# FauxFaux/quadrs

Hardware: AMD Instinct MI355X
Metric: Msamples/s through shift->FIR->FFT chain (higher is better)
Workload: dtype f32

## Files before the change

quadrs_amd/csrc/qd_chain.h:

```cpp
#pragma once

#include "qd_device.h"
#include "qd_geometry.h"

namespace qd {

#ifdef QD_STAMP
#define QD_STAMP_DECL unsigned long long st_prev = 0, st_acc[8] = {0, 0, 0, 0, 0, 0, 0, 0}, st_row[4] = {0, 0, 0, 0}; unsigned st_tiles = 0;
#define QD_STAMP_ROW(k) do { unsigned long long t_; asm volatile("s_memtime %0\n\ts_waitcnt lgkmcnt(0)" : "=s"(t_) :: "memory"); st_row[k] += t_ - st_prev; st_acc[0] += t_ - st_prev; st_prev = t_; } while (0)
#define QD_STAMP_START() do { asm volatile("s_memtime %0\n\ts_waitcnt lgkmcnt(0)" : "=s"(st_prev) :: "memory"); } while (0)
#define QD_STAMP_AT(k) do { unsigned long long t_; asm volatile("s_memtime %0\n\ts_waitcnt lgkmcnt(0)" : "=s"(t_) :: "memory"); st_acc[k] += t_ - st_prev; st_prev = t_; } while (0)
#define QD_STAMP_FLUSH() do { if (P.stamps && (threadIdx.x & 63) == 0 && threadIdx.x < 1024) { unsigned w_ = threadIdx.x >> 6; for (int k_ = 0; k_ < 8; ++k_) atomicAdd(&P.stamps[w_ * 8 + k_], st_acc[k_]); if (w_ == 1) for (int k_ = 0; k_ < 4; ++k_) atomicAdd(&P.stamps[129 + k_], st_row[k_]); if (w_ == 0) for (int k_ = 0; k_ < 4; ++k_) atomicAdd(&P.stamps[133 + k_], st_row[k_]); if (w_ == 0) atomicAdd(&P.stamps[128], (unsigned long long)st_tiles); } } while (0)
#define QD_STAMP_TILE() do { ++st_tiles; } while (0)
#else
#define QD_STAMP_DECL
#define QD_STAMP_START()
#define QD_STAMP_AT(k)
#define QD_STAMP_FLUSH()
#define QD_STAMP_TILE()
#define QD_STAMP_ROW(k)
#endif

#ifdef QD_BAKED_TAPS_LIST
constexpr float kBakedTapTable[] = {QD_BAKED_TAPS_LIST};
// ... 60 lines not shown
template <class GeoT>
__device__ __forceinline__ uint8_t glyph_of(const ChainParams &P, float nm) {
    if constexpr (GeoT::kFixed) return glyph_code(nm, P.rmin, P.rmax, P.gstep, P.rgstep);
    else return glyph_code_ieee(nm, P.rmin, P.rmax, P.gstep);
}

template <class GeoT>
__device__ __forceinline__ float2 win_mul(const ChainParams &P, uint32_t k, float2 v) {
    if constexpr (GeoT::kWindow) { const float wv = P.window[k]; v.x = v.x * wv; v.y = v.y * wv; }
    return v;
}
template <class GeoT>
__device__ __forceinline__ float win_mul(const ChainParams &P, uint32_t k, float v) {
    if constexpr (GeoT::kWindow) v = v * P.window[k];
    return v;
}


typedef float v2f __attribute__((ext_vector_type(2)));

template <uint32_t W_, uint32_t S_, uint32_t D_, uint32_t T_, uint32_t G_, uint32_t FIRB_ = 8, uint32_t FIRR_ = 1, uint32_t PAD_ = 1, uint32_t BATCH_ = 1,
          uint32_t FLAGS_ = 0>
struct FixedGeo {
    static constexpr bool kFixed = true;
    static constexpr bool kRows = false;
    static constexpr FixedRules R = fixed_rules(W_, S_, D_, T_, G_, FIRB_, FIRR_, PAD_, BATCH_, FLAGS_);
    static constexpr uint32_t kFlags = FLAGS_;
    static constexpr bool kWindow = (FLAGS_ & kGeoWindow) != 0;
    static constexpr uint32_t DpP = R.DpP;
    static constexpr uint32_t plane_floats = R.plane_floats;
    static constexpr bool planar_geometry = R.planar_geometry;
    static constexpr bool baked_request = R.baked_request;
    static constexpr uint32_t kBatch = R.kBatch;
    static constexpr uint32_t kFirBlock = R.kFirBlock;
    static constexpr bool kFirTile4 = R.kFirTile4;
    static constexpr uint32_t kFirTile = R.kFirTile;
    static constexpr uint32_t PD = R.PD;
    static constexpr uint32_t pshift = R.pshift;
    __device__ __forceinline__ explicit FixedGeo(const ChainParams &) {}
    static constexpr uint32_t W = W_, S = S_, D = D_, T = T_, G = G_;
    static constexpr uint32_t G_ct = G_, W_ct = W_;
    static constexpr uint32_t logW = R.logW;
    static constexpr uint32_t kPad = R.kPad;
    static constexpr uint32_t Dp = R.Dp;
    static constexpr uint32_t dshift = R.dshift;
    static constexpr uint32_t dmagic = R.dmagic;
    static constexpr uint32_t c = R.c;
    static constexpr uint32_t a0 = R.a0, b0 = R.b0;
    static constexpr uint32_t T_fast = R.T_fast;
    static constexpr uint32_t a1 = R.a1, b1 = R.b1;
    static constexpr uint32_t log_base = R.log_base;
    static constexpr uint32_t base_len = R.base_len;
    static constexpr uint32_t layers = R.layers;
    static constexpr bool kHalfTile = R.kHalfTile;
    static constexpr uint32_t kHalfOut = R.kHalfOut;
    static constexpr uint32_t kHalfRaw = R.kHalfRaw;
    static constexpr uint32_t lds_raw_elems_std = R.lds_raw_elems_std;
    static constexpr uint32_t kNtrunc = R.kNtrunc;
    static constexpr bool kShared = R.kShared;
    static constexpr bool split_ok(uint32_t nt) { return R.split_ok(nt); }
    static constexpr bool helper_ok(uint32_t nt) { return R.helper_ok(nt); }
    static constexpr bool split_ok_shared(uint32_t nt) { return R.split_ok_shared(nt); }
    static constexpr bool kPairFir = R.kPairFir;
    static constexpr bool kUnrolledShared = R.kUnrolledShared;
    static constexpr bool kPackedTile = R.kPackedTile;
    static constexpr bool kPlanar = R.kPlanar;
    static constexpr bool kBakedTaps = R.kBakedTaps;
    static constexpr uint32_t lds_raw_elems = R.lds_raw_elems;
};

struct DynGeo {
    static constexpr bool kFixed = false;
    static constexpr bool kRows = false;
    static constexpr bool kWindow = false;
    static constexpr uint32_t kBatch = 1;
    static constexpr uint32_t kFlags = 0, G_ct = 1, W_ct = 1;
    static constexpr bool kPlanar = false, kBakedTaps = false, kPairFir = false, kUnrolledShared = false, kPackedTile = false, kHalfTile = false;
    static constexpr uint32_t kHalfOut = 0, kHalfRaw = 0;
    static constexpr uint32_t DpP = 0, plane_floats = 0;
    static constexpr bool kShared = false;
    static constexpr uint32_t kFirTile = 1;
    static constexpr bool split_ok(uint32_t) { return false; }
    static constexpr bool helper_ok(uint32_t) { return false; }
    static constexpr bool split_ok_shared(uint32_t) { return false; }
    uint32_t W, S, D, T, G, logW, Dp, kPad, dshift, dmagic, PD, pshift, a0, b0, T_fast, a1, b1, log_base, base_len, layers, lds_raw_elems;
    __device__ __forceinline__ explicit DynGeo(const ChainParams &P)
        : W(P.W), S(P.S), D(P.D), T(P.T), G(P.G), logW(P.logW), Dp(P.Dp), kPad(P.Dp - P.D), dshift(P.dshift), dmagic(P.dmagic), PD(P.D), pshift(P.dshift),
          a0(P.a0), b0(P.b0), T_fast(P.T_fast), a1(P.a1), b1(P.b1), log_base(P.log_base), base_len(P.base_len),
          layers(P.layers), lds_raw_elems(P.lds_raw_elems) {}
};

struct WinGeo : DynGeo {
    static constexpr bool kWindow = true;
    __device__ __forceinline__ explicit WinGeo(const ChainParams &P) : DynGeo(P) {}
};

struct RowGeo : DynGeo {
    static constexpr bool kRows = true;
    __device__ __forceinline__ explicit RowGeo(const ChainParams &P) : DynGeo(P) {}
};


struct TileGeo {
    uint64_t w0, n_start;
    uint64_t r0;
    int64_t row0_off;
    int32_t slab_lo0, slab_hi0;
    uint32_t n_rows;
// ... 919 lines not shown
            float2 *d = fbp + (size_t)chunk * 4 * cols + i;
            float2 s0 = d[0];
            float2 s1 = cmul(d[cols], tw[3 * i]);
            float2 s2 = cmul(d[2 * cols], tw[3 * i + 1]);
            float2 s3 = cmul(d[3 * cols], tw[3 * i + 2]);
            bf4(s0, s1, s2, s3);
            d[0] = s0; d[cols] = s1; d[2 * cols] = s2; d[3 * cols] = s3;
        }
        tw += 3 * cols;
        cols *= 4;
        log_cols += 2;
    }
    wsync();
    if constexpr (PART == 3) return;
    const uint64_t wrel = pw0 - P.out_window0;
    const uint32_t n_out_s = pg << geo.logW;
    if (P.epi == 2) {
        constexpr uint32_t K = KB ? KB : (GeoT::kFixed ? (GeoT::G_ct * GeoT::W_ct + 63) / 64 : 1);
        wave_bucket_epilogue_fn<GeoT, K>(P, geo, fbp, pw0, pg, lane);
    } else if (P.epi == 4) {
        wave_mark_epilogue_fn<GeoT>(P, geo, [&](uint32_t o) { return fbp[o]; }, reinterpret_cast<uint8_t *>(P.out) + wrel, pg, lane);
    } else {
        float *outf = reinterpret_cast<float *>(P.out) + (wrel << geo.logW);
        uint8_t *outb = reinterpret_cast<uint8_t *>(P.out) + (wrel << geo.logW);
        for (uint32_t o = lane; o < n_out_s; o += 64) {
            const float2 xv = fbp[o ^ (geo.W >> 1)];
            const float nm = norm_ref(xv);
            if (P.epi == 0) outf[o] = nm;
            else outb[o] = glyph_of<GeoT>(P, nm);
        }
    }
}

template <class GeoT, bool HAS_FIR>
constexpr bool defer_fft_ok(uint32_t nt) {
    if constexpr (!GeoT::kFixed) return false;
    else return GeoT::R.defer_fft_ok(HAS_FIR, nt);
}

template <class GeoT, bool HAS_FIR>
constexpr bool quad_fft_ok(uint32_t nt) {
    if constexpr (!GeoT::kFixed) return false;
    else return GeoT::R.quad_fft_ok(HAS_FIR, nt);
}

template <int FMT, int NT, class GeoT>
constexpr bool fast_p1_ok(int rch, bool whole, bool aligned) {
    if constexpr (!GeoT::kFixed) return false;
    else return GeoT::R.fast_p1_ok(NT, FmtTraits<FMT>::SPL, (uint64_t)rch, whole, aligned);
}

template <int FMT, int NCO, class GeoT, bool HAS_FIR, int RCH, bool WHOLE, bool ALIGNED, int LB, int NT = kThreads>
__global__ __launch_bounds__(NT, LB) void k_chain(const ChainParams P) {
    using FT = FmtTraits<FMT>;
    using Vec = typename FT::Vec;
    constexpr int SPL = FT::SPL;
    constexpr bool HAS_SHIFT = NCO != 0;
    const GeoT geo(P);

    extern __shared__ __attribute__((aligned(16))) char smem[];
    float2 *raw = reinterpret_cast<float2 *>(smem);
    constexpr bool kDefer = defer_fft_ok<GeoT, HAS_FIR>((uint32_t)NT);
    constexpr bool kQuadFft = quad_fft_ok<GeoT, HAS_FIR>((uint32_t)NT);
    constexpr uint32_t kSlots = GeoT::kBatch;
    constexpr uint32_t kBatch = kDefer ? 1u : GeoT::kBatch;
    constexpr uint32_t kLutElems = (FMT == 1 || FMT == 2) ? 256u : 0u;
    float2 *fb0 = raw + geo.lds_raw_elems;
    float2 *twl = fb0 + (size_t)kSlots * geo.G * geo.W;
    float *tapl = reinterpret_cast<float *>(twl + geo.W);
    float *lut = tapl + ((GeoT::kBakedTaps && NT == 256) ? 0u : ((geo.T + 3) & ~3u));
    float2 *dec = reinterpret_cast<float2 *>(lut + kLutElems);
    float2 *trc = dec + ((geo.G - 1) * geo.S + geo.W);
    uint32_t *bmeta = reinterpret_cast<uint32_t *>(GeoT::kShared ? trc + ((geo.G - 1) * geo.S + geo.W) : dec);
    uint32_t *wq = bmeta + 4 * kSlots;

    const uint32_t tid = threadIdx.x;
    const uint32_t W = geo.W, logW = geo.logW, S = geo.S, D = geo.D, T = geo.T, Dp = geo.Dp;


    constexpr bool kReloadLane = HAS_SHIFT && ((GeoT::kFixed && GeoT::kFirTile > 1) || !GeoT::kFixed);
    constexpr bool kFastP1 = fast_p1_ok<FMT, NT, GeoT>(RCH, WHOLE, ALIGNED);
    constexpr bool kHalf = GeoT::kHalfTile;
    static_assert(!kHalf || (kFastP1 && defer_fft_ok<GeoT, HAS_FIR>((uint32_t)NT)), "half-window tiles: row-aligned phase 1 and the deferred FFT");
    static_assert((GeoT::kFlags & kGeoWindow) == 0 || (GeoT::kFixed && family_of(GeoT::kFlags) == kFamChain), "kGeoWindow: a plan-time build of k_chain");
    static_assert(!GeoT::kWindow || HAS_FIR || GeoT::kFixed, "WinGeo: behind a lowpass only (without one DynGeo tests the pointer)");
    uint32_t half = 0;
    LaneRot lr[SPL];
    auto load_lane_rot = [&](uint32_t first) {
#pragma unroll
        for (int u = 0; u < SPL; ++u) {
            uint32_t j = first + u;
            double2 cs = P.jtab[j];
            lr[u].jf = (double)j;
            lr[u].c = cs.x;
            lr[u].s = cs.y;
        }
    };
// ... 34 lines not shown
        asm volatile("" : "+s"(mx));
        const uint64_t dyn_base = 2 * walk_step;
        if (got + dyn_base < xcd_limit(mx)) return (uint64_t)mx * n8 + dyn_base + got;
#pragma unroll 1
        for (uint32_t k = 1; k < 8; ++k) {
            const uint32_t xx = (mx + k) & 7u;
            const uint64_t lim = xcd_limit(xx);
            if (lim <= dyn_base) continue;
            const unsigned long long i = atomicAdd(&P.work[16 * xx], 1ull);
            if (i + dyn_base < lim) return (uint64_t)xx * n8 + dyn_base + i;
        }
        return n_tiles;
    };
    uint64_t tile, tile_n;
    tile = walk_tile(walk_local);
    tile_n = walk_tile(walk_local + walk_step);
    TileGeo tg = tile_geo<FMT, NT>(P, geo, tile, n_tiles);
    Vec pf[RCH];
    if constexpr (!GeoT::kRows) {
    if (tg.valid) {
#pragma unroll
        for (int i = 0; i < RCH; ++i) pf[i] = fetch_row<FMT, NT, ALIGNED, (GeoT::kFlags & kGeoNtLoads) != 0>(P, tg, (uint32_t)i < tg.n_rows ? i : tg.n_rows - 1, tid);
    }
    }

#ifdef QD_WGTIME
    unsigned long long wg_t0 = __builtin_amdgcn_s_memrealtime();
#endif
    double rt_touch = 0.0;
    uint32_t dpar = 0, dprev_gcnt = 0;
    uint64_t dprev_w0 = 0;
    bool dprev_valid = false;
    auto wave_fft_epilogue = [&](float2 *fbp, uint64_t pw0, uint32_t pg) { wave_fft_epilogue_fn<GeoT>(P, geo, twl, fbp, pw0, pg, tid); };
    auto parks_norms = [](uint32_t epi) { return epi == 2 || (!GeoT::kFixed && epi == 4); };
    uint32_t quad_gen = 0;
    auto quad_fft_epilogue = [&](float2 *fbp, uint64_t pw0, uint32_t v) {
        uint32_t lane = tid & 63u;
        asm volatile("" : "+v"(lane));
        auto wsync = [] { __builtin_amdgcn_fence(__ATOMIC_ACQ_REL, "wavefront"); __builtin_amdgcn_wave_barrier(); };
        const uint32_t Wq = geo.W >> 2, base = geo.base_len;
        float2 *sub = fbp + (size_t)v * Wq;
        for (uint32_t t = lane; t < Wq / base; t += 64) {
            float2 *d = sub + (size_t)t * base;
            if (base == 16) {
                float2 x[16];
#pragma unroll
                for (int i = 0; i < 16; ++i) x[i] = d[i];
                bf16(x, P.tw16_1, P.tw16_2, P.tw16_3, P.root2);
#pragma unroll
                for (int i = 0; i < 16; ++i) d[i] = x[i];
            } else {
                float2 x[8];
#pragma unroll
                for (int i = 0; i < 8; ++i) x[i] = d[i];
                bf8(x, P.root2);
#pragma unroll
                for (int i = 0; i < 8; ++i) d[i] = x[i];
            }
        }
        uint32_t cols = base, log_cols = geo.log_base;
        const float2 *tw = twl;
        for (uint32_t layer = 0; layer + 1 < geo.layers; ++layer) {
            wsync();
            for (uint32_t t = lane; t < Wq / 4; t += 64) {
                const uint32_t chunk = t >> log_cols, i = t & (cols - 1);
                float2 *d = sub + (size_t)chunk * 4 * cols + i;
// ... 147 lines not shown
#pragma unroll
                for (int i = 0; i < RCH; ++i) cur[i] = pf[i];
                TileGeo ng = tg;
                uint32_t rbase = r + RCH;
                if (rbase >= tg.n_rows) {
                    const TileGeo t2 = tile_geo<FMT, NT>(P, geo, tile_n, n_tiles);
                    if (t2.valid) { ng = t2; rbase = 0; rt_pf = prefetch_rowtab<HAS_SHIFT>(P, t2, tid); } else { rbase = tg.n_rows - 1; }
                }
#pragma unroll
                for (int i = 0; i < RCH; ++i)
                    pf[i] = fetch_row<FMT, NT, ALIGNED, (GeoT::kFlags & kGeoNtLoads) != 0>(P, ng, rbase + i < ng.n_rows ? rbase + i : ng.n_rows - 1, tid);
                RowBase rb[RCH];
#pragma unroll
                for (int i = 0; i < RCH; ++i) {
                    rb[i] = RowBase{};
                    if constexpr (HAS_SHIFT) { if (r + i < tg.n_rows) rb[i] = load_rowbase(P, tg.r0 + r + i); }
                }
#pragma unroll
                for (int i = 0; i < RCH; ++i)
                    if (r + i < tg.n_rows) process_row_any<FMT, NT, NCO>(P, geo, tg, r + i, tid, cur[i], rb[i], lr, lane_pad, lut, raw);
            }
        }
        QD_STAMP_AT(0);
        __syncthreads();
        QD_STAMP_AT(1);

        __builtin_amdgcn_s_setprio(1);
        if constexpr (kDefer) {
            constexpr uint32_t GW = GeoT::G_ct * GeoT::W_ct, GWP = kHalf ? GeoT::kHalfOut : GW, FL = GeoT::kPackedTile ? GWP / 2 : GWP;
            float2 *fb_cur = fb0 + (size_t)dpar * GW, *fb_prev = fb0 + (size_t)(dpar ^ 1u) * GW;
            const uint32_t n_out_d = kHalf ? GWP : (g_cnt << logW);
            const uint32_t log_width_d = 2 * geo.layers;
            const uint32_t k_first = kHalf ? half * GWP : 0u;
            if (tid < FL) {
                if constexpr (GeoT::kPackedTile) {
                    const uint32_t o0 = tid * 2;
                    if (o0 < n_out_d) {
                        const uint32_t g = kHalf ? 0u : (o0 >> logW), k0 = kHalf ? k_first + o0 : (o0 & (W - 1));
                        uint32_t jm[2];
#pragma unroll
                        for (int r = 0; r < 2; ++r) { const uint32_t j2 = (W - (k0 + r)) * D + T / 2; jm[r] = j2 < T ? j2 : T; }
                        float2 full[2], snp[2];
                        const uint32_t q0 = kHalf ? o0 : g * S + k0;
                        if ((tid >> 8) & 1u) fir_tiled2_pk<GeoT, 1>(raw + (q0 * D + GeoT::kPad * (q0 / 2)), tapl, full, jm, snp); else fir_tiled2_pk<GeoT, 0>(raw + (q0 * D + GeoT::kPad * (q0 / 2)), tapl, full, jm, snp);
#pragma unroll
                        for (int r = 0; r < 2; ++r) {
                            const uint32_t k = k0 + r;
                            const uint32_t xx = k & ((1u << log_width_d) - 1), yy = k >> log_width_d;
                            fb_cur[(g << logW) + yy + (rev4(xx, geo.layers) << geo.log_base)] = win_mul<GeoT>(P, k, jm[r] < T ? snp[r] : full[r]);
                        }
                    }
                } else if (tid < n_out_d) {
                    const uint32_t g = kHalf ? 0u : (tid >> logW), k = kHalf ? k_first + tid : (tid & (W - 1));
                    uint32_t jmax = (W - k) * D + T / 2;
                    if (jmax > T) jmax = T;
                    const float2 *rp = raw + (size_t)((kHalf ? tid : g * S + k) + geo.a0) * Dp;
                    const float2 v = QD_DBG(P, 2) ? rp[0] : fir_pair<GeoT>(rp, jmax, tapl);
                    const uint32_t xx = k & ((1u << log_width_d) - 1), yy = k >> log_width_d;
                    fb_cur[(g << logW) + yy + (rev4(xx, geo.layers) << geo.log_base)] = win_pair(k, v);
                }
            } else if (kHalf && half != 0) {
            } else if (kQuadFft && !one_wave_sink(P.epi)) {
                if ((tid >> 6) < FL / 64 + 4 && dprev_valid) {
                    __builtin_amdgcn_s_setprio(3);
                    quad_fft_epilogue(fb_prev, dprev_w0, (tid >> 6) - FL / 64);
                }
            } else if ((tid >> 6) == FL / 64 && dprev_valid) {
                __builtin_amdgcn_s_setprio(3);
                wave_fft_epilogue(fb_prev, dprev_w0, dprev_gcnt);
            }
            QD_STAMP_AT(2);
            if constexpr (kHalf) {
                if (half == 0) {
                    __syncthreads();
                    QD_STAMP_AT(3);
                    half = 1;
                    rt_touch += rt_pf;
                    continue;
                }
                half = 0;
            }
            if (dyn && tid == 0) {
                const uint64_t t2 = claim_resolve(claim);
                wq[0] = (uint32_t)t2; wq[1] = (uint32_t)(t2 >> 32);
            }
            const TileGeo tg_nx = tile_geo<FMT, NT>(P, geo, tile_n, n_tiles);
            __syncthreads();
            QD_STAMP_AT(3);
            dprev_w0 = w0; dprev_gcnt = g_cnt; dprev_valid = true; dpar ^= 1u;
            tile = tile_n;
            if (dyn) tile_n = ((uint64_t)__builtin_amdgcn_readfirstlane(wq[1]) << 32) | __builtin_amdgcn_readfirstlane(wq[0]);
            else { walk_local += walk_step; tile_n = walk_tile(walk_local + walk_step); }
            rt_touch += rt_pf;
            tg = tg_nx;
            QD_STAMP_TILE();
            continue;
        }
        float2 *fb = fb0 + (size_t)bslot * geo.G * geo.W;
        const uint32_t n_out = g_cnt << logW;
        const uint32_t log_width = 2 * geo.layers;
        const bool cf32_out = !GeoT::kFixed && P.epi == 3;
        const uint32_t c_half = T - T / 2;
        const uint32_t ntrunc = c_half ? (c_half + D - 1) / D - 1 : 0;
        bool shared;
        if constexpr (GeoT::kFixed) shared = GeoT::kShared; else shared = HAS_FIR && S < W && ntrunc <= S && !QD_DBG(P, 2) && P.epi != 3;
        if constexpr (!GeoT::kFixed || GeoT::kShared) if (shared) {
            const uint32_t Q = (g_cnt - 1) * S + W;
            if constexpr (GeoT::kFixed && GeoT::kFirTile > 1) {
                constexpr int R = (int)GeoT::kFirTile;
                for (uint32_t q0 = tid * R; q0 < Q; q0 += NT * R) {
                    uint32_t jm[R];
#pragma unroll
                    for (int r = 0; r < R; ++r) {
                        const uint32_t qi = q0 + r;
                        jm[r] = T;
                        if (qi + ntrunc >= W) {
                            const uint32_t g = (qi - (W - ntrunc)) / S, k = qi - g * S;
                            if (k < W && g < g_cnt) { const uint32_t j2 = (W - k) * D + T / 2; if (j2 < T) jm[r] = j2; }
                        }
                    }
                    float2 full[R], snp[R];
                    fir_tiled<R, GeoT>(raw + (q0 * D + GeoT::kPad * (q0 / R)), jm, tapl, full, snp);
// ... 290 lines not shown
                asm volatile("" : "+v"(tt));
                reinterpret_cast<uint8_t *>(P.out)[wrel + tt] = (GeoT::kFixed || P.epi == 2) ? (first < second ? 0 : 1) : (mark ? 1 : 0);
            }
        } else if (GeoT::kFixed && P.epi == 4) {
            uint32_t ln = tid & 63u;
            asm volatile("" : "+v"(ln));
            wave_mark_epilogue_fn<GeoT>(P, geo, [&](uint32_t o) { return fbs[o]; }, reinterpret_cast<uint8_t *>(P.out) + wrel, n_out_s >> logW, ln,
                                        __builtin_amdgcn_readfirstlane(tid >> 6), NT / 64);
        } else {
            float *outf = reinterpret_cast<float *>(P.out) + (wrel << logW);
            uint8_t *outb = reinterpret_cast<uint8_t *>(P.out) + (wrel << logW);
            for (uint32_t o = tid; o < n_out_s; o += NT) {
                uint32_t oi = o;
                asm volatile("" : "+v"(oi));
                const float2 xv = fbs[oi ^ (W >> 1)];
                const float nm = QD_DBG(P, 8) ? xv.x : norm_ref(xv);
                uint32_t oo = o;
                asm volatile("" : "+v"(oo));
                if (QD_DBG(P, 16)) { asm volatile("" :: "v"(nm)); continue; }
                if (P.epi == 0) outf[oo] = nm;
                else outb[oo] = glyph_of<GeoT>(P, nm);
            }
        }
        }
        rt_touch += rt_pf;
        QD_STAMP_AT(6);
        if (parks_norms(P.epi)) __syncthreads();
        QD_STAMP_AT(7);
        QD_STAMP_TILE();
        tg = tg_next;
    }
    if constexpr (kDefer) {
        constexpr uint32_t GW = GeoT::G_ct * GeoT::W_ct, GWP = kHalf ? GeoT::kHalfOut : GW, FL = GeoT::kPackedTile ? GWP / 2 : GWP;
        if (kQuadFft && !one_wave_sink(P.epi)) {
            if (dprev_valid && (tid >> 6) >= FL / 64 && (tid >> 6) < FL / 64 + 4) quad_fft_epilogue(fb0 + (size_t)(dpar ^ 1u) * GW, dprev_w0, (tid >> 6) - FL / 64);
        } else
        if (dprev_valid && (tid >> 6) == FL / 64) wave_fft_epilogue(fb0 + (size_t)(dpar ^ 1u) * GW, dprev_w0, dprev_gcnt);
    }
    if (dyn && tid == 0) {
        if (atomicAdd(&P.work[16 * 8], 1ull) == (unsigned long long)gridDim.x - 1) {
#pragma unroll
            for (int x = 0; x <= 8; ++x) P.work[16 * x] = 0;
        }
    }
    QD_STAMP_FLUSH();
#ifdef QD_WGTIME
    if (P.stamps && tid == 0) {
        unsigned xcc;
        asm volatile("s_getreg_b32 %0, hwreg(HW_REG_XCC_ID)" : "=s"(xcc));
        unsigned long long *w = P.stamps + 256 + 4ull * blockIdx.x;
        w[0] = wg_t0; w[1] = __builtin_amdgcn_s_memrealtime(); w[2] = xcc & 0xf; w[3] = 1;
    }
#endif
    if (P.dbg == 0xdeadbeefu) reinterpret_cast<double *>(P.out)[tid] = rt_touch;
}

template <int V> struct IntC { static constexpr int value = V; };

template <int FMT, class GeoT>
constexpr bool pipe_geometry_ok(int rch) {
    if constexpr (!GeoT::kFixed) return false;
    else return GeoT::R.pipe_geometry_ok(FmtTraits<FMT>::SPL, (uint64_t)rch);
}

template <int FMT, int NCO, class GeoT, int RCH, int LB, int NT = kPipeThreads>
__global__ __launch_bounds__(NT, LB) void k_chain_pipe(const ChainParams P) {
// ... 1509 lines not shown
```

quadrs_amd/csrc/qd_geometry.h:

```cpp
#pragma once

#if !defined(__HIPCC_RTC__)
#include <stdint.h>
#else
typedef unsigned char uint8_t; typedef signed char int8_t; typedef unsigned short uint16_t; typedef short int16_t;
typedef unsigned int uint32_t; typedef int int32_t; typedef unsigned long long uint64_t; typedef long long int64_t;
#endif

namespace qd {

constexpr uint32_t kGeoPlanar = 1;
constexpr uint32_t kGeoBakedTaps = 2;
constexpr uint32_t kGeoNoSplit = 4;
constexpr uint32_t kGeoFastP1 = 8;
constexpr uint32_t kGeoPackedSpan = 16;
constexpr uint32_t kGeoUnrolledFir = 32;
constexpr uint32_t kGeoDeferFft = 64;
constexpr uint32_t kGeoPackedTile = 128;
constexpr uint32_t kGeoNtLoads = 256;
constexpr uint32_t kGeoPipe = 512;
constexpr uint32_t kGeoPipeFftWave = 1024;
constexpr uint32_t kGeoLoadSc0 = 2048;
constexpr uint32_t kGeoLoadSc1 = 4096;
constexpr uint32_t kGeoHalfTile = 8192;
// ... 44 lines not shown
}

constexpr uint32_t ct_log2(uint64_t v) { uint32_t l = 0; while ((1ull << l) < v) ++l; return l; }
constexpr bool ct_pow2(uint64_t v) { return v && !(v & (v - 1)); }
constexpr uint64_t ct_min(uint64_t a, uint64_t b) { return a < b ? a : b; }
constexpr uint64_t ct_max(uint64_t a, uint64_t b) { return a > b ? a : b; }
constexpr uint64_t ct_gcd(uint64_t a, uint64_t b) { while (b) { const uint64_t t = a % b; a = b; b = t; } return a; }
constexpr uint64_t ct_rows(uint64_t samples, uint64_t row) { return (samples + row - 1) / row; }
constexpr uint64_t ct_taps_bytes(uint64_t T) { return ((T + 3) & ~3ull) * 4; }

constexpr uint64_t ct_tile_elems(uint64_t tile_raw, uint64_t D, uint64_t GW, uint64_t pad_per_row) {
    const uint64_t pad = (D % 2 == 0) ? pad_per_row * (tile_raw / D + 1) : 0;
    return (ct_max(tile_raw + pad + 1, GW / 2 + 1) + 1) & ~1ull;
}
constexpr uint64_t ct_tile_raw(uint64_t W, uint64_t S, uint64_t D, uint64_t T, uint64_t G) { return (G - 1) * S * D + W * D + T; }
constexpr uint64_t ct_raw_elems(uint64_t W, uint64_t S, uint64_t D, uint64_t T, uint64_t G, uint64_t pad_per_row = 1) {
    return ct_tile_elems(ct_tile_raw(W, S, D, T, G), D, G * W, pad_per_row);
}
constexpr uint64_t ct_planar_pitch(uint64_t D) { return ((D / 4) % 2 == 1) ? D : D + 4; }
constexpr uint64_t ct_plane_floats(uint64_t W, uint64_t S, uint64_t D, uint64_t T, uint64_t G) {
    return ((ct_tile_raw(W, S, D, T, G) / D + 1) * ct_planar_pitch(D) + 7) & ~7ull;
}

struct FixedRules {
    uint64_t W, S, D, T, G;
    uint32_t flags, kBatch, kFirBlock;
    uint64_t DpP, plane_floats;
    bool planar_geometry, baked_request, kFirTile4;
    uint32_t kFirTile, pshift, logW, kPad, dshift, dmagic, log_base, base_len, layers;
    uint64_t PD, Dp, c, a0, b0, T_fast, a1, b1;
    bool kHalfTile;
    uint64_t kHalfOut, kHalfRaw, tile_raw, pass_raw, lds_raw_elems_std, kNtrunc, Q;
    bool kShared, kPairFir, kUnrolledShared, kPackedTile, kPlanar, kBakedTaps;
    uint64_t lds_raw_elems;
    uint64_t lds_raw_alloc;
    constexpr bool split_ok(uint64_t nt) const {
        return !(flags & kGeoNoSplit) && !kShared && kFirTile == 1 && kPad != 2 && D % 8 == 0 && T >= 64 && 2 * G * W <= nt;
    }
    constexpr bool helper_ok(uint64_t nt) const {
        return kFirTile > 1 && !kShared && (G * W / kFirTile) % 64 == 0 && G * W / kFirTile + G * kNtrunc <= nt &&
               (T / 2) % 8 == 0 && kNtrunc > 0 && kNtrunc < W;
    }
    constexpr bool split_ok_shared(uint64_t nt) const {
        return kShared && kFirTile == 1 && kPad != 2 && D % 8 == 0 && T >= 64 && 2 * Q <= nt;
    }
    constexpr uint64_t fir_lanes() const { return (kHalfTile ? kHalfOut : G * W) / (kPackedTile ? 2 : 1); }
    constexpr bool defer_fft_ok(bool has_fir, uint64_t nt) const {
        return has_fir && (kPairFir || kPackedTile) && (flags & kGeoDeferFft) != 0 && kBatch == 2 && fir_lanes() % 64 == 0 && fir_lanes() + 64 <= nt;
    }
    constexpr bool quad_fft_ok(bool has_fir, uint64_t nt) const {
        return defer_fft_ok(has_fir, nt) && G == 1 && W >= 256 && layers >= 1 && base_len >= 8 && fir_lanes() + 4 * 64 <= nt;
    }
    constexpr uint64_t rows(uint64_t nt, uint64_t spl) const { return ct_rows(pass_raw, nt * spl); }
    constexpr bool fast_p1_ok(uint64_t nt, uint64_t spl, uint64_t rch, bool whole, bool aligned) const {
        return whole && aligned && ((kHalfTile ? kHalfOut : S) * D) % (nt * spl) == 0 && (G * S * D) % (nt * spl) == 0 && rch == rows(nt, spl) &&
               D % spl == 0 && (flags & kGeoFastP1);
    }
    constexpr bool pipe_geometry_ok(uint64_t spl, uint64_t rch) const {
        return G == 1 && S == W && kPairFir && W == 128 && (S * D) % (256 * spl) == 0 && rch == ct_rows(W * D + T, 256 * spl) && D % spl == 0 && T > D;
    }
    constexpr bool pipe3_geometry_ok(uint64_t spl, uint64_t rch) const {
        return kShared && kUnrolledShared && Q <= 256 && (G * S * D) % (kPipe3Prod * spl) == 0 && rch == ct_rows(tile_raw, kPipe3Prod * spl) &&
               D % spl == 0 && W <= 64 * 16 && G >= 1;
    }
    constexpr uint64_t pipe3_q_pad() const { return (Q + 1) & ~1ull; }
    constexpr bool spark2_ok() const {
        return (base_len == 8 || base_len == 16) && layers >= 1 && (W / base_len == 16 || W / base_len == 64) && S <= W && S >= 1 && D == 1 && T == 0;
    }
    constexpr bool spark0_ok(uint64_t bps) const {
        return W >= 2 && W <= 16 && S >= 1 && S <= W && D == 1 && T == 0 && (W * bps) % 4 == 0 && (S * bps) % 4 == 0;
    }
};

constexpr FixedRules fixed_rules(uint64_t W, uint64_t S, uint64_t D, uint64_t T, uint64_t G, uint32_t firb = 8, uint32_t firr = 1, uint32_t pad = 1,
                                 uint32_t batch = 1, uint32_t flags = 0) {
    FixedRules r{};
    r.W = W; r.S = S; r.D = D; r.T = T; r.G = G; r.flags = flags;
    r.kBatch = batch ? batch : 1;
    r.kFirBlock = firb;
    r.c = T - T / 2;
    r.tile_raw = ct_tile_raw(W, S, D, T, G);
// ... 1 lines not shown
    r.DpP = ct_planar_pitch(D);
    r.plane_floats = ct_plane_floats(W, S, D, T, G);
    r.planar_geometry = (flags & kGeoPlanar) && ct_pow2(D) && D % 8 == 0 && T % 4 == 0 && (r.c % D) % 4 == 0 && T >= 64 && ct_pow2(G * W);
    r.baked_request = (flags & kGeoBakedTaps) != 0;
    r.kFirTile4 = firr == 2 && (flags & kGeoPackedTile) && pad == 2 && D % 4 == 0 && r.c % 4 == 0 && T % 4 == 0 && (T / 2) % 4 == 0 && W % 2 == 0 && S % 2 == 0 &&
                  ct_pow2(D) && D / 4 <= 8 && T > D + 16 && !(T > 0 && S < W);
    r.kFirTile = r.kFirTile4 ? 2u
               : (firr > 1 && D % 8 == 0 && (r.c % D) % 8 == 0 && T % 8 == 0 && (T / 2) % 8 == 0 && W % firr == 0 && S % firr == 0 && ct_pow2(D) && ct_pow2(firr) &&
                  T > (uint64_t)(firr - 1) * D + 8) ? firr : 1u;
    r.PD = D * r.kFirTile;
    r.pshift = ct_pow2(r.PD) ? ct_log2(r.PD) : 0xffffffffu;
    r.logW = ct_log2(W);
    r.kPad = (D % 2 == 0) ? ((pad == 2 && r.c % 2 == 0) ? 2u : 1u) : 0u;
    r.Dp = D + r.kPad;
    r.dshift = ct_pow2(D) ? ct_log2(D) : 0xffffffffu;
    r.dmagic = D > 1 ? (uint32_t)((1ull << 32) / D + 1) : 0u;
    r.a0 = r.c / D; r.b0 = r.c % D;
    r.T_fast = ct_min(T, D + T / 2);
    r.a1 = (r.c + r.T_fast) / D; r.b1 = (r.c + r.T_fast) % D;
    r.log_base = r.logW <= 3 ? r.logW : ((r.logW & 1) ? 3u : 4u);
    r.base_len = 1u << r.log_base;
    r.layers = (r.logW - r.log_base) / 2;
    r.kHalfTile = (flags & kGeoHalfTile) && G == 1 && !(T > 0 && S < W) && W % 4 == 0 && T > 0;
    r.kHalfOut = W / 2;
    r.kHalfRaw = r.c + (r.kHalfOut - 1) * D + T;
    r.pass_raw = r.kHalfTile ? r.kHalfRaw : r.tile_raw;
    r.lds_raw_elems_std = ct_tile_elems(r.pass_raw, D, G * W, r.kPad ? r.kPad : 1);
    r.kNtrunc = r.c ? (r.c + D - 1) / D - 1 : 0;
    r.kShared = T > 0 && S < W && r.kNtrunc <= S;
    const bool pair_geo = r.kFirTile == 1 && r.kPad == 2 && T % 4 == 0 && r.b0 % 2 == 0 && D % 4 == 0 && T >= 32;
    r.kPairFir = (flags & kGeoNoSplit) && !r.kShared && pair_geo;
    r.kUnrolledShared = (flags & kGeoUnrolledFir) && r.kShared && pair_geo;
    r.kPackedTile = (flags & kGeoPackedTile) && !r.kShared && r.kFirTile == 2 && r.kPad == 2 && (T / 2) % 4 == 0 && D / 4 <= 8;
    r.kPlanar = r.planar_geometry && r.split_ok(256);
    r.kBakedTaps = r.baked_request && r.kPlanar;
    r.lds_raw_elems = r.kPlanar ? r.plane_floats : r.lds_raw_elems_std;
    r.lds_raw_alloc = ct_max(ct_tile_elems(r.pass_raw, D, G * W, pad), ((flags & kGeoPlanar) && r.pass_raw < (1u << 24)) ? r.plane_floats : 0);
    return r;
}

struct Pipe3sRules {
    uint64_t SPL, ROW, N, RN, GS, f0, RR, RINGD, MIRD, ROWP, RAW_ELEMS, DR, FBX_OFF, FBX_ALIGN, kLdsBytes, GH;
    bool kOverlap, fir_ok, ok, kWrite, kSwzFft;
    uint32_t kConsumerThreads;
};
constexpr Pipe3sRules pipe3s_rules(uint64_t spl, uint64_t pt, const FixedRules &g) {
    Pipe3sRules k{};
    const uint64_t W = g.W, S = g.S, D = g.D, T = g.T, G = g.G;
    k.SPL = spl; k.ROW = pt * spl;
    k.N = G * S * D; k.RN = k.N / k.ROW; k.GS = G * S;
    k.f0 = k.N >= g.c + T ? (k.N - g.c - T) / D + 1 : 0;
    k.RR = (2 * k.N + T + 2 * D + k.ROW - 1) / k.ROW;
    k.RINGD = k.RR * (k.ROW / D);
    k.MIRD = (g.b0 + T + D - 1) / D + 1;
    k.ROWP = (k.ROW / D) * g.Dp;
    k.RAW_ELEMS = ((k.RINGD + k.MIRD) * g.Dp + 1) & ~1ull;
    k.DR = 3 * k.GS;
    k.kOverlap = S < W;
    k.fir_ok = k.kOverlap ? (g.kShared && g.kUnrolledShared)
                          : (S == W && g.kPad == 2 && T % 4 == 0 && g.b0 % 2 == 0 && D % 4 == 0 && T / 4 > 3 && (T / 2) % 4 == 0);
    k.ok = k.fir_ok && k.GS <= 256 && k.GS >= 1 && k.N % k.ROW == 0 && k.ROW % D == 0 && D % spl == 0 && W <= 64 * 16 && k.f0 >= 1 && k.f0 <= k.GS &&
           k.f0 > W - S && g.kNtrunc <= S && k.MIRD * D <= k.ROW && g.Q <= 2 * k.GS;
    k.kWrite = (g.flags & kGeoWriteSink) != 0;
    const uint64_t rings = k.RAW_ELEMS + (k.kOverlap ? 2u : 1u) * k.DR;
    k.FBX_OFF = (rings + 31u) & ~31ull;
    k.FBX_ALIGN = k.FBX_OFF - rings;
    k.kLdsBytes = k.kWrite ? k.RAW_ELEMS * 8 + ct_taps_bytes(T) : (k.FBX_OFF + 2 * G * W + W) * 8 + ct_taps_bytes(T);
    k.GH = (G + 1) / 2;
    k.kSwzFft = !k.kWrite && W >= 8 && (k.GH * W) % 32 == 0 && (G * W) % 32 == 0;
    k.kConsumerThreads = k.kWrite ? 256u : 512u;
    return k;
}

constexpr uint64_t chain_lds_bytes(const FixedRules &g, bool lut8) {
    const bool baked = g.baked_request && (g.flags & kGeoPlanar) && g.pass_raw < (1u << 24);
    return g.lds_raw_alloc * 8 + g.kBatch * g.G * g.W * 8 + g.W * 8 + (baked ? 0 : ct_taps_bytes(g.T)) + (lut8 ? 256 * 4 : 0) +
           ((g.T && g.S < g.W) ? 2 * g.Q * 8 : 0) + g.kBatch * 16 + 16;
}
constexpr uint64_t generic_raw_elems(const FixedRules &g) { return ct_tile_elems(g.tile_raw, g.D, g.G * g.W, 1); }
constexpr uint64_t generic_lds_bytes(const FixedRules &g, bool lut8) {
    return generic_raw_elems(g) * 8 + g.G * g.W * 8 + g.W * 8 + ct_taps_bytes(g.T) + (lut8 ? 256 * 4 : 0) + ((g.T && g.S < g.W) ? 2 * g.Q * 8 : 0) + 16 + 16;
}
constexpr uint64_t kPipe3QueueBytes = 8;
constexpr uint64_t pipe3_lds_bytes(const FixedRules &g) {
    return 2 * g.lds_raw_alloc * 8 + 4 * g.pipe3_q_pad() * 8 + g.G * g.W * 8 + g.W * 8 + ct_taps_bytes(g.T) + kPipe3QueueBytes;
}
constexpr uint64_t spark_lds_bytes(uint64_t W, uint64_t ts, bool lane_table) { return (ct_max(W, 32) + 4 * ts) * 8 + (lane_table ? kSparkRow * 16 : 0); }
constexpr uint64_t kPipe3LdsSlack = 64 - kPipe3QueueBytes, kStreamLdsSlack = 320, kStreamWriteLdsSlack = 64;
static_assert(31 * 8 < kStreamLdsSlack, "the streaming layout's slack covers FBX_OFF's rounding");

}
```

quadrs_amd/csrc/quadrs_hip.hip:

```cpp
#include <hip/hip_runtime.h>
#include <hip/hiprtc.h>

#include <dlfcn.h>
#include <map>
#include <cmath>
#include <cstdarg>
#include <cstdio>
#include <cstring>
#include <cstdlib>
#include <functional>
#include <memory>
#include <mutex>
#include <numeric>
#include <optional>
#include <thread>
#include <algorithm>
#include <sys/stat.h>
#include <time.h>
#include <unistd.h>
#include <tuple>
#include <string>
#include <vector>

#include "../../include/quadrs_hip.h"
// ... 303 lines not shown
}

typedef void (*blue_fn)(const BlueSrc, const uint64_t *, const float *, uint32_t, uint32_t, uint32_t, const double2 *, const double2 *, const double2 *, float *);
template <int F>
blue_fn pick_blue_fmt(int nco) { return nco == 0 ? k_bluestein<F, 0> : (nco == 1 ? k_bluestein<F, 1> : k_bluestein<F, 2>); }
blue_fn pick_blue(int fmt, int nco) {
#define QD_X(F) pick_blue_fmt<F>(nco)
    switch (fmt) { QD_FMT_CASES(QD_X) }
#undef QD_X
    return nullptr;
}

template <int F, int TS>
chain_fn pick_spark_ts(int nco) {
    constexpr int NCH = TS / (int)SparkTraits<F>::CH;
    switch (nco) {
    case 0: return k_spark<F, 0, DynGeo, NCH, 4>;
    case 1: return k_spark<F, 1, DynGeo, NCH, (TS == 512 ? 3 : 2)>;
    default: return k_spark<F, 2, DynGeo, NCH, 2>;
    }
}
int spark_lb(uint32_t ts, int nco) { return nco == 0 ? 4 : (nco == 1 && ts == 512 ? 3 : 2); }
uint32_t spark_tile(uint32_t W, int nco) { return (nco != 0 && W <= 512) ? 512u : 1024u; }
chain_fn pick_spark(int fmt, int nco, uint32_t ts) {
#define QD_X(F) (ts == 512 ? pick_spark_ts<F, 512>(nco) : pick_spark_ts<F, 1024>(nco))
    switch (fmt) { QD_FMT_CASES(QD_X) }
#undef QD_X
    return nullptr;
}

const FixedEntry kFixed[] = {
    QD_FIXED_FB(0, 1, 128, 128, 16, 40, 2, 9, true, 4, 1, 1, 65800, "cfg2"),
    QD_FIXED_FB(0, 2, 128, 128, 16, 40, 2, 9, true, 4, 1, 1, 65800, "cfg2"),
    QD_FIXED_FB(0, 1, 128, 128, 32, 200, 1, 9, true, 4, 2, 2, 65868, "cfg3p"),
    QD_FIXED_FB(0, 2, 128, 128, 32, 200, 1, 9, true, 4, 2, 2, 65868, "cfg3p"),
    { 0, 1, 64, 16, 32, 400, 14, 4, 512, 2, 1, 164128,
      qd::k_chain_pipe3s<0, 1, qd::FixedGeo<64, 16, 32, 400, 14, 8, 1, 2, 1, 164128>, 7, 4>, "fsk5" },
    { 0, 2, 64, 16, 32, 400, 14, 4, 512, 2, 1, 164128,
      qd::k_chain_pipe3s<0, 2, qd::FixedGeo<64, 16, 32, 400, 14, 8, 1, 2, 1, 164128>, 7, 4>, "fsk5" },
#ifndef QD_DEV_FAST
    { 1, 1, 64, 16, 32, 400, 14, 4, 256, 2, 1, 164128,
      qd::k_chain_pipe3s<1, 1, qd::FixedGeo<64, 16, 32, 400, 14, 8, 1, 2, 1, 164128>, 7, 4, 256>, "cfg3" },
    { 1, 2, 64, 16, 32, 400, 14, 4, 256, 2, 1, 164128,
      qd::k_chain_pipe3s<1, 2, qd::FixedGeo<64, 16, 32, 400, 14, 8, 1, 2, 1, 164128>, 7, 4, 256>, "cfg3" },
#endif
    { 0, 0, 1024, 1024, 8, 512, 1, 4, 512, 2, 2, 8392,
      qd::k_chain<0, 0, qd::FixedGeo<1024, 1024, 8, 512, 1, 4, 2, 2, 2, 8392>, true, 5, true, true, 4, 512>, "cfg4" },
};

const FixedEntry *find_fixed(int fmt, int nco, uint32_t W, uint32_t S, uint32_t D, uint32_t T) {
    for (const FixedEntry &e : kFixed)
        if (e.fmt == fmt && e.nco == nco && e.W == W && e.S == S && e.D == D && e.T == T) return &e;
    return nullptr;
}

struct JitKey {
    int fmt, nco, fir, rch, whole, lb, nt; uint32_t W, S, D, T, G; uint32_t firb = 8, firr = 1; int noslp = 0; uint32_t pad = 1, batch = 1, flags = 0;
    uint64_t taps_hash = 0;
    int epi = 0;
    bool operator<(const JitKey &o) const {
        return std::tie(fmt, nco, fir, rch, whole, lb, nt, W, S, D, T, G, firb, firr, noslp, pad, batch, flags, taps_hash, epi) <
               std::tie(o.fmt, o.nco, o.fir, o.rch, o.whole, o.lb, o.nt, o.W, o.S, o.D, o.T, o.G, o.firb, o.firr, o.noslp, o.pad, o.batch, o.flags, o.taps_hash, o.epi);
    }
};
std::mutex g_jit_mu;
std::map<std::pair<int, JitKey>, hipFunction_t> g_jit_cache;
std::map<std::pair<int, JitKey>, std::string> g_jit_failed;

std::string csrc_dir() {
    Dl_info info;
    if (!dladdr(reinterpret_cast<const void *>(&csrc_dir), &info) || !info.dli_fname) return "";
    std::string path(info.dli_fname);
    size_t slash = path.rfind('/');
    return (slash == std::string::npos ? std::string(".") : path.substr(0, slash)) + "/csrc";
}

uint64_t fnv1a(const void *data, size_t n, uint64_t h = 1469598103934665603ull) {
    const unsigned char *p = static_cast<const unsigned char *>(data);
    for (size_t i = 0; i < n; ++i) { h ^= p[i]; h *= 1099511628211ull; }
    return h;
}
// ... 3788 lines not shown
```

Measured before the change: 629,500.

## Pair deferred FFTs so the spare wave transforms two windows per launch

Adds a paired deferred-FFT mode for small-width, single-group chain geometries. FIR lanes park their windowed output in registers and write it into one of two FFT slots after the barrier. A spare wave runs the FFT and norm epilogue on two parked windows at once at raised priority, instead of one window every tile. The cfg3p built-in entries switch the batch parameter to select this mode while keeping the same LDS budget. This halves how often the spare wave runs the FFT and amortizes its cost, at the price of extra register state and latency, plus a flush at the end of the kernel.

```diff
diff --git a/quadrs_amd/csrc/qd_chain.h b/quadrs_amd/csrc/qd_chain.h
--- a/quadrs_amd/csrc/qd_chain.h
+++ b/quadrs_amd/csrc/qd_chain.h
@@ -116,6 +116,9 @@
     static constexpr bool planar_geometry = R.planar_geometry;
     static constexpr bool baked_request = R.baked_request;
     static constexpr uint32_t kBatch = R.kBatch;
+    static constexpr bool kPairFft = R.kPairFft;
+    static constexpr uint32_t kFftSlots = R.fft_slots;
+    static_assert(fixed_rules(W_, S_, D_, T_, G_, 8, 1, PAD_, BATCH_, FLAGS_).fft_slots == R.fft_slots, "the host sizes the FFT slots without FIRB_ / FIRR_ (lds_for)");
     static constexpr uint32_t kFirBlock = R.kFirBlock;
     static constexpr bool kFirTile4 = R.kFirTile4;
     static constexpr uint32_t kFirTile = R.kFirTile;
@@ -157,7 +160,8 @@
     static constexpr bool kFixed = false;
     static constexpr bool kRows = false;
     static constexpr bool kWindow = false;
-    static constexpr uint32_t kBatch = 1;
+    static constexpr uint32_t kBatch = 1, kFftSlots = 1;
+    static constexpr bool kPairFft = false;
     static constexpr uint32_t kFlags = 0, G_ct = 1, W_ct = 1;
     static constexpr bool kPlanar = false, kBakedTaps = false, kPairFir = false, kUnrolledShared = false, kPackedTile = false, kHalfTile = false;
     static constexpr uint32_t kHalfOut = 0, kHalfRaw = 0;
@@ -1143,6 +1147,20 @@
     }
 }
 
+template <class GeoT>
+__device__ __forceinline__ void wave_fft_pair_fn(const ChainParams &P, const GeoT &geo, const float2 *twl, float2 *fbp, uint64_t pw0, uint64_t pw1, uint32_t tid) {
+    wave_fft_epilogue_fn<GeoT, 0, 3>(P, geo, twl, fbp, pw0, 2u, tid);
+    uint32_t lane = tid & 63u;
+    asm volatile("" : "+v"(lane));
+#pragma unroll
+    for (uint32_t g = 0; g < 2; ++g) {
+        const uint64_t wrel = (g ? pw1 : pw0) - P.out_window0;
+        float *outf = reinterpret_cast<float *>(P.out) + (wrel << geo.logW);
+        const float2 *fw = fbp + ((size_t)g << geo.logW);
+        for (uint32_t o = lane; o < geo.W; o += 64) outf[o] = norm_ref(fw[o ^ (geo.W >> 1)]);
+    }
+}
+
 template <class GeoT, bool HAS_FIR>
 constexpr bool defer_fft_ok(uint32_t nt) {
     if constexpr (!GeoT::kFixed) return false;
@@ -1173,7 +1191,9 @@
     float2 *raw = reinterpret_cast<float2 *>(smem);
     constexpr bool kDefer = defer_fft_ok<GeoT, HAS_FIR>((uint32_t)NT);
     constexpr bool kQuadFft = quad_fft_ok<GeoT, HAS_FIR>((uint32_t)NT);
-    constexpr uint32_t kSlots = GeoT::kBatch;
+    constexpr bool kPair = kDefer && GeoT::kPairFft;
+    static_assert(!GeoT::kPairFft || kDefer, "paired deferred FFT: a spare wave beside the FIR's (the layout has two slots, not a batch of three)");
+    constexpr uint32_t kSlots = GeoT::kFftSlots;
     constexpr uint32_t kBatch = kDefer ? 1u : GeoT::kBatch;
     constexpr uint32_t kLutElems = (FMT == 1 || FMT == 2) ? 256u : 0u;
     float2 *fb0 = raw + geo.lds_raw_elems;
@@ -1274,6 +1294,13 @@
     uint64_t dprev_w0 = 0;
     bool dprev_valid = false;
     auto wave_fft_epilogue = [&](float2 *fbp, uint64_t pw0, uint32_t pg) { wave_fft_epilogue_fn<GeoT>(P, geo, twl, fbp, pw0, pg, tid); };
+    uint32_t npark = 0;
+    uint64_t park_w0 = 0, park_w1 = 0;
+    const uint32_t pair_lim = P.epi == 0 ? 2u : 1u;
+    auto wave_fft_parked = [&] {
+        if (npark == 2) wave_fft_pair_fn<GeoT>(P, geo, twl, fb0, park_w0, park_w1, tid);
+        else wave_fft_epilogue_fn<GeoT>(P, geo, twl, fb0, park_w0, 1u, tid);
+    };
     auto parks_norms = [](uint32_t epi) { return epi == 2 || (!GeoT::kFixed && epi == 4); };
     uint32_t quad_gen = 0;
     auto quad_fft_epilogue = [&](float2 *fbp, uint64_t pw0, uint32_t v) {
@@ -1487,6 +1514,8 @@
             const uint32_t n_out_d = kHalf ? GWP : (g_cnt << logW);
             const uint32_t log_width_d = 2 * geo.layers;
             const uint32_t k_first = kHalf ? half * GWP : 0u;
+            float2 park_v = make_float2(0.f, 0.f);
+            uint32_t park_pos = 0;
             if (tid < FL) {
                 if constexpr (GeoT::kPackedTile) {
                     const uint32_t o0 = tid * 2;
@@ -1512,7 +1541,14 @@
                     const float2 *rp = raw + (size_t)((kHalf ? tid : g * S + k) + geo.a0) * Dp;
                     const float2 v = QD_DBG(P, 2) ? rp[0] : fir_pair<GeoT>(rp, jmax, tapl);
                     const uint32_t xx = k & ((1u << log_width_d) - 1), yy = k >> log_width_d;
-                    fb_cur[(g << logW) + yy + (rev4(xx, geo.layers) << geo.log_base)] = win_pair(k, v);
+                    const uint32_t pos = (g << logW) + yy + (rev4(xx, geo.layers) << geo.log_base);
+                    if constexpr (kPair) { park_v = win_pair(k, v); park_pos = pos; }
+                    else fb_cur[pos] = win_pair(k, v);
+                }
+            } else if (kPair) {
+                if ((tid >> 6) == FL / 64 && npark == pair_lim) {
+                    __builtin_amdgcn_s_setprio(3);
+                    wave_fft_parked();
                 }
             } else if (kHalf && half != 0) {
             } else if (kQuadFft && !one_wave_sink(P.epi)) {
@@ -1542,7 +1578,12 @@
             const TileGeo tg_nx = tile_geo<FMT, NT>(P, geo, tile_n, n_tiles);
             __syncthreads();
             QD_STAMP_AT(3);
-            dprev_w0 = w0; dprev_gcnt = g_cnt; dprev_valid = true; dpar ^= 1u;
+            if constexpr (kPair) {
+                if (npark == pair_lim) npark = 0;
+                if (tid < FL) fb0[npark * GW + park_pos] = park_v;
+                if (npark == 0) park_w0 = w0; else park_w1 = w0;
+                ++npark;
+            } else { dprev_w0 = w0; dprev_gcnt = g_cnt; dprev_valid = true; dpar ^= 1u; }
             tile = tile_n;
             if (dyn) tile_n = ((uint64_t)__builtin_amdgcn_readfirstlane(wq[1]) << 32) | __builtin_amdgcn_readfirstlane(wq[0]);
             else { walk_local += walk_step; tile_n = walk_tile(walk_local + walk_step); }
@@ -1899,6 +1940,10 @@
     }
     if constexpr (kDefer) {
         constexpr uint32_t GW = GeoT::G_ct * GeoT::W_ct, GWP = kHalf ? GeoT::kHalfOut : GW, FL = GeoT::kPackedTile ? GWP / 2 : GWP;
+        if constexpr (kPair) {
+            __syncthreads();
+            if (npark != 0 && (tid >> 6) == FL / 64) wave_fft_parked();
+        } else
         if (kQuadFft && !one_wave_sink(P.epi)) {
             if (dprev_valid && (tid >> 6) >= FL / 64 && (tid >> 6) < FL / 64 + 4) quad_fft_epilogue(fb0 + (size_t)(dpar ^ 1u) * GW, dprev_w0, (tid >> 6) - FL / 64);
         } else
diff --git a/quadrs_amd/csrc/qd_geometry.h b/quadrs_amd/csrc/qd_geometry.h
--- a/quadrs_amd/csrc/qd_geometry.h
+++ b/quadrs_amd/csrc/qd_geometry.h
@@ -100,6 +100,8 @@
     bool kHalfTile;
     uint64_t kHalfOut, kHalfRaw, tile_raw, pass_raw, lds_raw_elems_std, kNtrunc, Q;
     bool kShared, kPairFir, kUnrolledShared, kPackedTile, kPlanar, kBakedTaps;
+    bool kPairFft;
+    uint32_t fft_slots;
     uint64_t lds_raw_elems;
     uint64_t lds_raw_alloc;
     constexpr bool split_ok(uint64_t nt) const {
@@ -114,7 +116,7 @@
     }
     constexpr uint64_t fir_lanes() const { return (kHalfTile ? kHalfOut : G * W) / (kPackedTile ? 2 : 1); }
     constexpr bool defer_fft_ok(bool has_fir, uint64_t nt) const {
-        return has_fir && (kPairFir || kPackedTile) && (flags & kGeoDeferFft) != 0 && kBatch == 2 && fir_lanes() % 64 == 0 && fir_lanes() + 64 <= nt;
+        return has_fir && (kPairFir || kPackedTile) && (flags & kGeoDeferFft) != 0 && (kBatch == 2 || kPairFft) && fir_lanes() % 64 == 0 && fir_lanes() + 64 <= nt;
     }
     constexpr bool quad_fft_ok(bool has_fir, uint64_t nt) const {
         return defer_fft_ok(has_fir, nt) && G == 1 && W >= 256 && layers >= 1 && base_len >= 8 && fir_lanes() + 4 * 64 <= nt;
@@ -182,6 +184,8 @@
     r.kPairFir = (flags & kGeoNoSplit) && !r.kShared && pair_geo;
     r.kUnrolledShared = (flags & kGeoUnrolledFir) && r.kShared && pair_geo;
     r.kPackedTile = (flags & kGeoPackedTile) && !r.kShared && r.kFirTile == 2 && r.kPad == 2 && (T / 2) % 4 == 0 && D / 4 <= 8;
+    r.kPairFft = r.kBatch == 3 && (flags & kGeoDeferFft) && family_of(flags) == kFamChain && r.kPairFir && G == 1 && !r.kHalfTile && W <= 128;
+    r.fft_slots = r.kPairFft ? 2u : r.kBatch;
     r.kPlanar = r.planar_geometry && r.split_ok(256);
     r.kBakedTaps = r.baked_request && r.kPlanar;
     r.lds_raw_elems = r.kPlanar ? r.plane_floats : r.lds_raw_elems_std;
@@ -224,8 +228,8 @@
 
 constexpr uint64_t chain_lds_bytes(const FixedRules &g, bool lut8) {
     const bool baked = g.baked_request && (g.flags & kGeoPlanar) && g.pass_raw < (1u << 24);
-    return g.lds_raw_alloc * 8 + g.kBatch * g.G * g.W * 8 + g.W * 8 + (baked ? 0 : ct_taps_bytes(g.T)) + (lut8 ? 256 * 4 : 0) +
-           ((g.T && g.S < g.W) ? 2 * g.Q * 8 : 0) + g.kBatch * 16 + 16;
+    return g.lds_raw_alloc * 8 + g.fft_slots * g.G * g.W * 8 + g.W * 8 + (baked ? 0 : ct_taps_bytes(g.T)) + (lut8 ? 256 * 4 : 0) +
+           ((g.T && g.S < g.W) ? 2 * g.Q * 8 : 0) + g.fft_slots * 16 + 16;
 }
 constexpr uint64_t generic_raw_elems(const FixedRules &g) { return ct_tile_elems(g.tile_raw, g.D, g.G * g.W, 1); }
 constexpr uint64_t generic_lds_bytes(const FixedRules &g, bool lut8) {
diff --git a/quadrs_amd/csrc/quadrs_hip.hip b/quadrs_amd/csrc/quadrs_hip.hip
--- a/quadrs_amd/csrc/quadrs_hip.hip
+++ b/quadrs_amd/csrc/quadrs_hip.hip
@@ -359,8 +359,8 @@
 const FixedEntry kFixed[] = {
     QD_FIXED_FB(0, 1, 128, 128, 16, 40, 2, 9, true, 4, 1, 1, 65800, "cfg2"),
     QD_FIXED_FB(0, 2, 128, 128, 16, 40, 2, 9, true, 4, 1, 1, 65800, "cfg2"),
-    QD_FIXED_FB(0, 1, 128, 128, 32, 200, 1, 9, true, 4, 2, 2, 65868, "cfg3p"),
-    QD_FIXED_FB(0, 2, 128, 128, 32, 200, 1, 9, true, 4, 2, 2, 65868, "cfg3p"),
+    QD_FIXED_FB(0, 1, 128, 128, 32, 200, 1, 9, true, 4, 2, 3, 65868, "cfg3p"),
+    QD_FIXED_FB(0, 2, 128, 128, 32, 200, 1, 9, true, 4, 2, 3, 65868, "cfg3p"),
     { 0, 1, 64, 16, 32, 400, 14, 4, 512, 2, 1, 164128,
       qd::k_chain_pipe3s<0, 1, qd::FixedGeo<64, 16, 32, 400, 14, 8, 1, 2, 1, 164128>, 7, 4>, "fsk5" },
     { 0, 2, 64, 16, 32, 400, 14, 4, 512, 2, 1, 164128,
@@ -374,6 +374,11 @@
     { 0, 0, 1024, 1024, 8, 512, 1, 4, 512, 2, 2, 8392,
       qd::k_chain<0, 0, qd::FixedGeo<1024, 1024, 8, 512, 1, 4, 2, 2, 2, 8392>, true, 5, true, true, 4, 512>, "cfg4" },
 };
+
+static_assert(fixed_rules(128, 128, 32, 200, 1, 8, 1, 2, 3, 65868).kPairFft && fixed_rules(128, 128, 32, 200, 1, 8, 1, 2, 3, 65868).defer_fft_ok(true, kThreads) &&
+              4 * chain_lds_bytes(fixed_rules(128, 128, 32, 200, 1, 8, 1, 2, 3, 65868), false) <= 160 * 1024 &&
+              chain_lds_bytes(fixed_rules(128, 128, 32, 200, 1, 8, 1, 2, 3, 65868), false) == chain_lds_bytes(fixed_rules(128, 128, 32, 200, 1, 8, 1, 2, 2, 65868), false),
+              "cfg3' built-in: paired deferred FFT, four workgroups per CU");
 
 const FixedEntry *find_fixed(int fmt, int nco, uint32_t W, uint32_t S, uint32_t D, uint32_t T) {
     for (const FixedEntry &e : kFixed)
```

After: 630,800 (median of 3 runs). About the same (+0.2%).
